# asmirnou/watsor

Measured on AMD Instinct MI355X. Metric: detected frames/sec (whole node) + p50 per-frame latency, SSD-MobileNet 300x300, higher is better.
Workload: dtype f16; 1 GPU; 1 synthetic 640x480 RGB stream per GPU, batch=8 frames, SSD-MobileNet-v2 300x300 (seeded random-init weights), frames resident in HBM, rows copied back to host; batch=8, frame=640x480, parallelism=replica-per-gpu x1, batches_in_flight=4, graph_nodes_per_batch=31

## Files before the change

### include/watsor_hip.h

```cpp
#ifndef WATSOR_HIP_H
#define WATSOR_HIP_H

#include <stdint.h>

#ifdef __cplusplus
extern "C" {
#endif

#define WZ_MAX_DETECTIONS 100
#define WZ_MAX_ZONES 10
#define WZ_NUM_LABELS 91
#define WZ_MAX_CAMS 256

#define WZ_OK 0
#define WZ_EINVAL (-1)
#define WZ_ENOENT (-2)
#define WZ_EFORMAT (-3)
#define WZ_EHIP (-4)
#define WZ_ENODEV (-5)
#define WZ_ELIMIT (-6)
#define WZ_EINCOMPLETE (-7)

typedef struct wz_detection {
    int32_t label;
// ... 102 lines not shown
int wz_input_size(wz_engine_t* e);
int wz_num_anchors(wz_engine_t* e);
int wz_num_classes(wz_engine_t* e);
int wz_precision(wz_engine_t* e);
int wz_hp_blocks(wz_engine_t* e);
double wz_nms_iou(wz_engine_t* e);

int wz_dev_alloc(wz_engine_t* e, uint64_t bytes, void** d_ptr);
int wz_dev_free(wz_engine_t* e, void* d_ptr);
int wz_dev_upload(wz_engine_t* e, void* d_dst, const void* h_src, uint64_t bytes);
int wz_dev_download(wz_engine_t* e, void* h_dst, const void* d_src, uint64_t bytes);

#ifdef WZ_DEV_BUILD
int wz_debug_pyset_order(const int32_t* keys, int n, int32_t* out);
int wz_debug_unused_order(int n, const uint8_t* used, int32_t* out);

int wz_num_tensors(wz_engine_t* e);
int wz_tensor_info(wz_engine_t* e, int idx, char* name, int namelen, int* h, int* w, int* c);
int wz_tensor_flags(wz_engine_t* e, int idx);
int wz_num_ops(wz_engine_t* e);
int wz_op_info(wz_engine_t* e, int idx, char* name, int namelen, int* dims);
int wz_num_stages(wz_engine_t* e);
int wz_stage_name(wz_engine_t* e, int stage, char* name, int namelen);
int wz_profile_device(wz_engine_t* e, int n, const uint8_t* const* d_rgb, const int* w, const int* h,
                      int reps, float* stage_ms);
int wz_profile_stages(wz_engine_t* e, int n, const uint8_t* const* d_rgb, const int* w, const int* h,
                      int reps, int inner, float* stage_ms);

int wz_debug_nms(wz_engine_t* e, int n, uint64_t* out);
int wz_debug_post_lane(wz_engine_t* e, int slot, int n, float* box_enc, float* logits, float* boxes, float* scores,
                       int32_t* classes, int32_t* num, uint64_t* dbg, int32_t* flags);
int wz_debug_mbconv(wz_engine_t* e, uint64_t* out, int32_t* groups);

int wz_debug_lane_stamps(wz_engine_t* e, int slot, uint64_t* out, int cap);
int wz_debug_lane_launch(wz_engine_t* e, int slot, int idx, char* name, int namelen, int* dims);

int wz_stage_preprocess(wz_engine_t* e, const uint8_t* rgb, int w, int h, uint16_t* out_half);
int wz_stage_preprocess_fmt(wz_engine_t* e, const uint8_t* frame, int w, int h, int fmt, uint16_t* out_half);
int wz_stage_forward(wz_engine_t* e, int n, const uint16_t* in_half, float* box_enc, float* logits);
int wz_stage_read_tensor(wz_engine_t* e, int idx, int frame, uint16_t* out_half);
int wz_stage_postprocess(wz_engine_t* e, int n, const float* box_enc, const float* logits, float* boxes,
                         float* scores, int32_t* classes, int32_t* num);
int wz_stage_post_production(wz_engine_t* e, int n, const float* box_enc, const float* logits, int w, int h, wz_detection_t* rows);
int wz_stage_rows(wz_engine_t* e, int w, int h, const float* boxes, const float* scores,
                  const int32_t* classes, wz_detection_t* rows);
int wz_stage_crop_tile(wz_engine_t* e, const uint8_t* frame, int w, int h, int fmt, const wz_tile_t* tile, uint8_t* out);
int wz_stage_merge_tiles(wz_engine_t* e, int w, int h, int cam, int n_tiles, const wz_tile_t* tiles,
                         const wz_detection_t* tile_rows , double iou_thr, double ios_thr,
                         wz_detection_t* rows , uint8_t* pass );
int wz_profile_tiled(wz_engine_t* e, int n, const uint8_t* const* d_frames, const int* w, const int* h, const int* fmt,
                     const int* n_tiles, const wz_tile_t* const* tiles, double iou_thr, double ios_thr, int reps,
                     float* crop_ms, float* merge_ms, float* empty_ms);
int wz_stage_tile_activity(wz_engine_t* e, const uint8_t* frame, int w, int h, int fmt, const wz_tile_t* tile, const uint16_t* ref, int pixel_thr,
                           uint16_t* sums_out, int32_t* changed_out);
int wz_profile_gated(wz_engine_t* e, int n, const uint8_t* const* d_frames, const int* w, const int* h, const int* fmt, const int* cam,
                     double iou_thr, double ios_thr, int reps, float* activity_ms, float* commit_ms, float* empty_ms);
int wz_debug_bound_source(wz_engine_t* e, int slot, int32_t* in_place );

#endif

#ifdef __cplusplus
}
#endif
#endif
```

### watsor_amd/_lib.py

```python
from __future__ import annotations

import ctypes as C
import os

from .share import Detection

_HERE = os.path.dirname(os.path.abspath(__file__))
LIB_PATH = os.path.join(_HERE, "libwatsor_hip.so")
DEV_LIB_PATH = os.environ.get("WATSOR_HIP_DEV_LIBRARY") or os.path.join(_HERE, "libwatsor_hip_dev.so")

WZ_OK, WZ_EINVAL, WZ_ENOENT, WZ_EFORMAT, WZ_EHIP, WZ_ENODEV, WZ_ELIMIT, WZ_EINCOMPLETE = 0, -1, -2, -3, -4, -5, -6, -7
WZ_SLOTS = 8
WZ_FMT_RGB24, WZ_FMT_NV12, WZ_FMT_I420 = 0, 1, 2
WZ_FMT_YUYV422, WZ_FMT_UYVY422, WZ_FMT_GRAY8, WZ_FMT_BGR24 = 3, 4, 5, 6
WZ_FMT_P010, WZ_FMT_YUV420P10 = 0x10, 0x11
WZ_FMT_BASE_MASK, WZ_CSP_BT709, WZ_RANGE_FULL = 0xFF, 0x100, 0x200
WZ_NUM_LABELS = 91
WZ_MAX_CAMS = 256
WZ_MAX_TILES = 64
WZ_GATE_CELL = 16
WZ_SCHEDULE_THROUGHPUT, WZ_SCHEDULE_LATENCY = 0, 1

c_u8p = C.POINTER(C.c_uint8)
c_i32p = C.POINTER(C.c_int32)
# ... 57 lines not shown
    "wz_tracker_count": (C.c_int, [C.c_void_p]),
    "wz_tracker_update": (C.c_int, [C.c_void_p, C.c_void_p, C.c_int, C.c_void_p, C.c_void_p, C.c_int,
                                    C.POINTER(C.c_int), C.POINTER(C.c_int)]),
    "wz_tracker_sieve": (C.c_int, [C.c_void_p, C.c_void_p, C.c_int, C.c_void_p, C.POINTER(C.c_int)]),
    "wz_zones_from_alpha": (C.c_int, [C.c_void_p, C.c_int, C.c_int, C.c_int, C.c_void_p, C.c_void_p]),
    "wz_input_size": (C.c_int, [C.c_void_p]),
    "wz_precision": (C.c_int, [C.c_void_p]),
    "wz_num_anchors": (C.c_int, [C.c_void_p]),
    "wz_num_classes": (C.c_int, [C.c_void_p]),
    "wz_hp_blocks": (C.c_int, [C.c_void_p]),
    "wz_nms_iou": (C.c_double, [C.c_void_p]),
    "wz_dev_alloc": (C.c_int, [C.c_void_p, C.c_uint64, C.POINTER(C.c_void_p)]),
    "wz_dev_free": (C.c_int, [C.c_void_p, C.c_void_p]),
    "wz_dev_upload": (C.c_int, [C.c_void_p, C.c_void_p, C.c_void_p, C.c_uint64]),
    "wz_dev_download": (C.c_int, [C.c_void_p, C.c_void_p, C.c_void_p, C.c_uint64]),
}

DEV_SIGNATURES = {
    "wz_debug_pyset_order": (C.c_int, [C.c_void_p, C.c_int, C.c_void_p]),
    "wz_debug_unused_order": (C.c_int, [C.c_int, C.c_void_p, C.c_void_p]),
    "wz_num_tensors": (C.c_int, [C.c_void_p]),
    "wz_tensor_info": (C.c_int, [C.c_void_p, C.c_int, C.c_char_p, C.c_int, c_i32p, c_i32p, c_i32p]),
    "wz_tensor_flags": (C.c_int, [C.c_void_p, C.c_int]),
    "wz_num_ops": (C.c_int, [C.c_void_p]),
    "wz_op_info": (C.c_int, [C.c_void_p, C.c_int, C.c_char_p, C.c_int, c_i32p]),
    "wz_num_stages": (C.c_int, [C.c_void_p]),
    "wz_stage_name": (C.c_int, [C.c_void_p, C.c_int, C.c_char_p, C.c_int]),
    "wz_profile_device": (C.c_int, [C.c_void_p, C.c_int, C.POINTER(C.c_void_p), c_i32p, c_i32p, C.c_int, c_f32p]),
    "wz_profile_stages": (C.c_int, [C.c_void_p, C.c_int, C.POINTER(C.c_void_p), c_i32p, c_i32p, C.c_int, C.c_int, c_f32p]),
    "wz_debug_nms": (C.c_int, [C.c_void_p, C.c_int, C.c_void_p]),
    "wz_debug_post_lane": (C.c_int, [C.c_void_p, C.c_int, C.c_int, C.c_void_p, C.c_void_p, C.c_void_p, C.c_void_p, C.c_void_p, C.c_void_p,
                                     C.c_void_p, C.c_void_p]),
    "wz_debug_mbconv": (C.c_int, [C.c_void_p, C.c_void_p, C.c_void_p]),
    "wz_debug_lane_stamps": (C.c_int, [C.c_void_p, C.c_int, C.c_void_p, C.c_int]),
    "wz_debug_lane_launch": (C.c_int, [C.c_void_p, C.c_int, C.c_int, C.c_char_p, C.c_int, c_i32p]),
    "wz_stage_preprocess": (C.c_int, [C.c_void_p, C.c_void_p, C.c_int, C.c_int, C.c_void_p]),
    "wz_stage_preprocess_fmt": (C.c_int, [C.c_void_p, C.c_void_p, C.c_int, C.c_int, C.c_int, C.c_void_p]),
    "wz_stage_forward": (C.c_int, [C.c_void_p, C.c_int, C.c_void_p, C.c_void_p, C.c_void_p]),
    "wz_stage_read_tensor": (C.c_int, [C.c_void_p, C.c_int, C.c_int, C.c_void_p]),
    "wz_stage_postprocess": (C.c_int, [C.c_void_p, C.c_int, C.c_void_p, C.c_void_p, C.c_void_p, C.c_void_p,
                                       C.c_void_p, C.c_void_p]),
    "wz_stage_post_production": (C.c_int, [C.c_void_p, C.c_int, C.c_void_p, C.c_void_p, C.c_int, C.c_int, C.c_void_p]),
    "wz_stage_rows": (C.c_int, [C.c_void_p, C.c_int, C.c_int, C.c_void_p, C.c_void_p, C.c_void_p, C.c_void_p]),
    "wz_stage_crop_tile": (C.c_int, [C.c_void_p, C.c_void_p, C.c_int, C.c_int, C.c_int, C.c_void_p, C.c_void_p]),
    "wz_profile_tiled": (C.c_int, [C.c_void_p, C.c_int, C.POINTER(C.c_void_p), c_i32p, c_i32p, c_i32p, c_i32p, C.POINTER(C.c_void_p),
                                   C.c_double, C.c_double, C.c_int, c_f32p, c_f32p, c_f32p]),
    "wz_stage_tile_activity": (C.c_int, [C.c_void_p, C.c_void_p, C.c_int, C.c_int, C.c_int, C.c_void_p, C.c_void_p, C.c_int, C.c_void_p,
                                         C.c_void_p]),
    "wz_profile_gated": (C.c_int, [C.c_void_p, C.c_int, C.POINTER(C.c_void_p), c_i32p, c_i32p, c_i32p, c_i32p, C.c_double, C.c_double, C.c_int,
                                   c_f32p, c_f32p, c_f32p]),
    "wz_debug_bound_source": (C.c_int, [C.c_void_p, C.c_int, C.c_void_p]),
    "wz_stage_merge_tiles": (C.c_int, [C.c_void_p, C.c_int, C.c_int, C.c_int, C.c_int, C.c_void_p, C.c_void_p, C.c_double, C.c_double,
                                       C.c_void_p, C.c_void_p]),
}

_lib = None
_dev_lib = None


class HipLibraryMissing(ImportError):
    pass


class RowsIncomplete(ValueError):
    """WZ_EINCOMPLETE: the call wrote every row, but a frame's rows may be short (clip-after-NMS engines).  The ONLY failure after
    which the rows are valid: callers that must tell "rows written" from "rows not written" catch this class, not ValueError."""
# ... 51 lines not shown
```

### watsor_amd/csrc/k_conv.hip

```cpp
#include "wz_common.h"

__global__ __launch_bounds__(256) void wz_k_stem(const half_t* __restrict__ in, const float* __restrict__ w,
                                                 const float* __restrict__ bias, half_t* __restrict__ out,
                                                 int total, int hin, int win, int hout, int wout, int pad_t,
                                                 int pad_l) {
    __shared__ float sw[27 * 32 + 32];
    for (int i = threadIdx.x; i < 27 * 32; i += 256) sw[i] = w[i];
    if (threadIdx.x < 32) sw[27 * 32 + threadIdx.x] = bias[threadIdx.x];
    __syncthreads();
    const int tid = blockIdx.x * 256 + threadIdx.x;
    if (tid >= total) return;
    const int cg = tid & 3, pix = tid >> 2;
    const int ox = pix % wout;
    const int t2 = pix / wout;
    const int oy = t2 % hout, b = t2 / hout;
    float acc[8];
#pragma unroll
    for (int j = 0; j < 8; ++j) acc[j] = sw[27 * 32 + cg * 8 + j];
#pragma unroll
    for (int ky = 0; ky < 3; ++ky) {
        const int iy = oy * 2 - pad_t + ky;
        if (iy < 0 || iy >= hin) continue;
#pragma unroll
        for (int kx = 0; kx < 3; ++kx) {
// ... 265 lines not shown
    for (int q = q0; q < q1;) {
        wz_conv_load<KS, MT, NT, U>(a, fb, ql, q1, t, c, iy0, ix0, boff, mv, wlane, nt0, cg8);
        wz_conv_mfma(fa, acc);
        q += U;
        if (q >= q1) break;
        wz_conv_load<KS, MT, NT, U>(a, fa, ql, q1, t, c, iy0, ix0, boff, mv, wlane, nt0, cg8);
        wz_conv_mfma(fb, acc);
        q += U;
    }

#pragma unroll
    for (int mt = 0; mt < MT; ++mt) {
        const int m = m_base + mt * 16 + r16;
#pragma unroll
        for (int nt = 0; nt < NT; ++nt) {
            const int n4 = (nt0 + nt) * 16 + g * 4;
            if (a.splitk > 1) {
                if (m < a.M)
                    *reinterpret_cast<float4_t*>(reinterpret_cast<float*>(a.out) +
                                                 ((size_t)bz * a.M + m) * a.n_pad + n4) = acc[mt][nt];
            } else {
                wz_epilogue4(a, m, n4, acc[mt][nt]);
            }
        }
    }
}

template <int KS, int MT, int NT, int U>
__global__ __launch_bounds__(256) void wz_k_conv(const WzConvArgs a) {
    WZ_LANE_STAMP(a.dbg);
    wz_conv_body<KS, MT, NT, U>(a, blockIdx.x, blockIdx.y, blockIdx.z);
}

template <int KS, int WM = 1, int WN = 1, int U = 2, int WGS_PER_CU = 2>
__global__ __launch_bounds__(512, WGS_PER_CU) void wz_k_conv_ws(const WzConvArgs a) {
    WZ_LANE_STAMP(a.dbg);
    constexpr int MT = 2, NT = 2, WAVES = 8, KSPL = WAVES / (WM * WN);
    static_assert(KSPL * WM * WN == WAVES, "eight waves: sub-tiles x K slices");
    __shared__ float4_t red[WAVES][MT * NT][64];
    const int lane = threadIdx.x & 63;
    const int wave = __builtin_amdgcn_readfirstlane(threadIdx.x >> 6);
    const int r16 = lane & 15, g = lane >> 4;
    const int sub = wave / KSPL, ks = wave - sub * KSPL;
    const int m_base = ((int)blockIdx.x * WM + sub / WN) * (MT * 16);
    const int nt0 = ((int)blockIdx.y * WN + sub % WN) * NT;
    const bool tile_live = m_base < a.M && nt0 * 16 < a.n_pad;

    const int hw = a.hout * a.wout;
    int iy0[MT], ix0[MT], boff[MT];
    bool mv[MT];
#pragma unroll
    for (int mt = 0; mt < MT; ++mt) {
        const int m = m_base + mt * 16 + r16;
        mv[mt] = m < a.M;
        const int mm = mv[mt] ? m : 0;
        const int b = mm / hw, rem = mm - b * hw;
        const int oy = rem / a.wout, ox = rem - oy * a.wout;
        iy0[mt] = oy * a.stride - a.pad_t;
        ix0[mt] = ox * a.stride - a.pad_l;
        boff[mt] = b * a.hin;
    }
    float4_t acc[MT][NT];
#pragma unroll
    for (int mt = 0; mt < MT; ++mt)
#pragma unroll
        for (int nt = 0; nt < NT; ++nt) acc[mt][nt] = (float4_t){0.f, 0.f, 0.f, 0.f};

    const int per = (a.kchunks + KSPL - 1) / KSPL;
    const int q0 = ks * per, q1 = min(q0 + per, a.kchunks);
    if (tile_live && q0 < q1) {
        const half_t* wlane = a.w + (size_t)lane * 8;
        const int cg8 = g * 8;
        int ql = q0, t = (KS == 1) ? 0 : q0 / a.kc, c = (KS == 1) ? q0 : q0 - t * a.kc;
        ConvFrags<MT, NT, U> fa, fb;
        wz_conv_load<KS, MT, NT, U>(a, fa, ql, q1, t, c, iy0, ix0, boff, mv, wlane, nt0, cg8);
        for (int q = q0; q < q1;) {
            wz_conv_load<KS, MT, NT, U>(a, fb, ql, q1, t, c, iy0, ix0, boff, mv, wlane, nt0, cg8);
            wz_conv_mfma(fa, acc);
            q += U;
            if (q >= q1) break;
            wz_conv_load<KS, MT, NT, U>(a, fa, ql, q1, t, c, iy0, ix0, boff, mv, wlane, nt0, cg8);
            wz_conv_mfma(fb, acc);
            q += U;
        }
    }
#pragma unroll
    for (int mt = 0; mt < MT; ++mt)
#pragma unroll
        for (int nt = 0; nt < NT; ++nt) red[wave][mt * NT + nt][lane] = acc[mt][nt];
    __syncthreads();
    if (tile_live) {
        for (int tl = ks; tl < MT * NT; tl += KSPL) {
            float4_t v = red[sub * KSPL][tl][lane];
#pragma unroll
            for (int z = 1; z < KSPL; ++z) {
                const float4_t p = red[sub * KSPL + z][tl][lane];
#pragma unroll
                for (int r = 0; r < 4; ++r) v[r] += p[r];
            }
            wz_epilogue4(a, m_base + (tl / NT) * 16 + r16, (nt0 + tl % NT) * 16 + g * 4, v);
        }
    }
}

__global__ __launch_bounds__(256) void wz_k_conv_group(const WzConvGroup g) {
    WZ_LANE_STAMP(g.stamp);
    int e = 0;
    while (e + 1 < g.n && (int)blockIdx.x >= g.first[e + 1]) ++e;
    const int L = (int)blockIdx.x - g.first[e];
    const int gx = g.gx[e], gy = g.gy[e];
    wz_conv_body<3, 2, 2, 4>(g.a[e], L % gx, (L / gx) % gy, L / (gx * gy));
}

__global__ __launch_bounds__(256) void wz_k_splitk_reduce(const WzConvArgs a, const float* __restrict__ ws) {
    WZ_LANE_STAMP(a.dbg);
    const int tid = blockIdx.x * 256 + threadIdx.x;
    const int n4s = a.n_pad >> 2;
// ... 138 lines not shown
void wz_launch_conv(const WzConvArgs& a0, hipStream_t s) {
    if (wz_conv_use_lds(a0)) {
        WzConvArgs a = a0;
        a.grid_m = (a.M + WZ_LDS_TM - 1) / WZ_LDS_TM;
        const int nw = wz_lds_nw(a.M, a.n_pad, a.kchunks);
        a.grid_n = (a.n_pad + WZ_LDS_TN(nw) - 1) / WZ_LDS_TN(nw);
        dim3 grid(a.grid_m * a.grid_n * a.splitk);
        if (nw == 4) {
            if (a.ksize == 1)
                wz_launch_conv_lds<1, 4>(a, grid, s);
            else
                wz_launch_conv_lds<3, 4>(a, grid, s);
        } else {
            if (a.ksize == 1)
                wz_launch_conv_lds<1, 2>(a, grid, s);
            else
                wz_launch_conv_lds<3, 2>(a, grid, s);
        }
        return;
    }
    const WzConvArgs& a = a0;
    if (wz_conv_big(a.M, a.n_pad, a.kchunks))
        wz_launch_conv_cfg<4, 4, 2>(a, s);
    else
        wz_launch_conv_cfg<2, 2, 4>(a, s);
}

bool wz_conv_ws_applies(const WzConvArgs& a) {
    static const int on = wz_dev_env_int("WZ_CONV_WS", 1);
    return on && a.out_mode == WZ_OUT_ACT && a.M <= 1024 && a.kchunks >= 8 && a.n_pad % 32 == 0;
}
void wz_launch_conv_ws(const WzConvArgs& a, hipStream_t s) {
    static const int wide_tiles = wz_dev_env_int("WZ_CONV_WS64", 1);
    if (wide_tiles && a.ksize == 1 && a.M >= 512 && a.n_pad >= 512 && a.n_pad % 64 == 0 && a.kchunks >= 8) {
        WZ_LAUNCH((wz_k_conv_ws<1, 1, 2>), dim3((a.M + 31) / 32, a.n_pad / 64), dim3(512), 0, s, a);
        return;
    }
    const dim3 grid((a.M + 31) / 32, a.n_pad / 32);
    if (a.ksize == 1)
        WZ_LAUNCH(wz_k_conv_ws<1>, grid, dim3(512), 0, s, a);
    else
        WZ_LAUNCH(wz_k_conv_ws<3>, grid, dim3(512), 0, s, a);
}

bool wz_conv_groupable(const WzConvArgs& a) {
    return a.ksize == 3 && !wz_conv_use_lds(a) && !wz_conv_big(a.M, a.n_pad, a.kchunks);
}
void wz_conv_group_add(WzConvGroup& g, const WzConvArgs& a) {
    const int i = g.n++;
    const int mtiles = (a.M + 31) / 32;
    g.a[i] = a;
    g.gx[i] = (mtiles + 3) / 4;
    g.gy[i] = a.n_pad / 32;
    g.first[i + 1] = g.first[i] + g.gx[i] * g.gy[i] * a.splitk;
    g.a[i].grid_m = g.gx[i];
    g.a[i].grid_n = g.gy[i];
}
void wz_launch_conv_group(const WzConvGroup& g, hipStream_t s) {
    WZ_LAUNCH(wz_k_conv_group, dim3(g.first[g.n]), dim3(256), 0, s, g);
}

bool wz_conv_rs_groupable(const WzConvArgs& a) {
    return a.ksize == 3 && wz_conv_use_lds(a);
}
int wz_conv_rs_group_add(WzConvGroup& g, const WzConvArgs& a0) {
    static const int split_n = wz_dev_env_int("WZ_HEAD_SPLIT_N", 1);
    const int nw = wz_lds_nw(a0.M, a0.n_pad, a0.kchunks);
    const bool two = split_n && nw == 4 && (a0.n_pad % 128) == 64 && a0.n_pad > 128;
    if (g.n + (two ? 2 : 1) > WZ_CONV_GROUP_MAX) return 0;
    for (int part = 0; part < (two ? 2 : 1); ++part) {
        const int i = g.n++;
// ... 32 lines not shown
```

### watsor_amd/csrc/k_mbconv_hp.hip

```cpp
#include "wz_common.h"

#include "k_hp_ops.h"

#ifndef WZ_HP_STAMPS
#define WZ_HP_STAMPS 0
#endif
#ifndef WZ_HP_RR3
#define WZ_HP_RR3 1
#endif
#ifndef WZ_HP_ROWS3
#define WZ_HP_ROWS3 1
#endif
#ifndef WZ_HP_STAMP_LAST
#define WZ_HP_STAMP_LAST 0
#endif

template <int NW, bool CS, bool STEM, int MPW, int MQW, int KCI, int NTO, int OCC = 2, bool ONEPASS = false, bool QE = false,
          bool LEAN = false>
__global__ __launch_bounds__(NW * 64, OCC) void wz_k_mbconv_hp(const WzMbArgs a) {
    static_assert(!LEAN || (CS && !ONEPASS && !STEM), "lean: chunk-split");
    static_assert(!LEAN || MQW == 1, "lean builds: 4 x 4 tiles (the 4 x 8 lean builds of round 5 lost their A/B: profiles/r05_blocks_13_16_tile_4x8.txt)");
    extern __shared__ __attribute__((aligned(16))) unsigned char wz_hp_smem[];
    WZ_LANE_STAMP(a.dbg);
    const long long t_entry = WZ_HP_STAMPS ? __builtin_readcyclecounter() : 0;
// ... 18 lines not shown
    const int bidx = (int)blockIdx.x;
    const int nt0 = LEAN ? (bidx % ngrp) * NTO : 0;
    const int wt = LEAN ? bidx / ngrp : CS ? (int)blockIdx.x : (int)blockIdx.x * 4 + __builtin_amdgcn_readfirstlane(wave);
    const bool live = wt < tiles * a.nb;
    const int wtc = live ? wt : 0;
    const int b = wtc / tiles, t = wtc - b * tiles;
    const int tyi = t / a.tiles_x;
    const int oy0 = tyi * a.th, ox0 = (t - tyi * a.tiles_x) * a.tw;
    const int s = a.stride;
    const int hw_ = (a.tw - 1) * s + 3, hh_ = (a.th - 1) * s + 3;
    const int P = hh_ * hw_;
    const int iy_base = oy0 * s - a.pad_t, ix_base = ox0 * s - a.pad_l;
    const half8_t zero8 = {0, 0, 0, 0, 0, 0, 0, 0};

    int hp0[MQW], opix[MQW];
#pragma unroll
    for (int j = 0; j < MQW; ++j) {
        int qy, qx;
        if constexpr (MQW == 2) {
            qx = r16 & 7;
            qy = ((r16 >> 3) << 1) + j;
        } else {
            qy = r16 >> 2;
            qx = r16 & 3;
        }
        hp0[j] = qy * s * hw_ + qx * s;
        const int oy = oy0 + qy, ox = ox0 + qx;
        opix[j] = (live && oy < a.hout && ox < a.wout) ? (b * a.hout + oy) * a.wout + ox : -1;
    }

    half8_t xh[MPW][KCI], xl[MPW][KCI];
    bool inimg[MPW];
    const float rcp_hw = 1.0f / (float)hw_;
#pragma unroll
    for (int i = 0; i < MPW; ++i) {
        const int p = i * 16 + r16;
        const int hy = (int)(((float)p + 0.5f) * rcp_hw), hx = p - hy * hw_;
        const int iy = iy_base + hy, ix = ix_base + hx;
        const bool ok = live && p < P && iy >= 0 && iy < a.hin && ix >= 0 && ix < a.win;
        inimg[i] = ok;
        if constexpr (STEM) {
            auto tap = [&](int tq, bool want) -> half8_t {
                const int ky = tq / 3, kx = tq - ky * 3;
                const int sy = iy * 2 - a.spad_t + ky, sx = ix * 2 - a.spad_l + kx;
                const bool in = want && ok && sy >= 0 && sy < a.sin_h && sx >= 0 && sx < a.sin_w;
                const int cy = min(max(sy, 0), a.sin_h - 1), cx = min(max(sx, 0), a.sin_w - 1);
                const half8_t v = *reinterpret_cast<const half8_t*>(a.in + ((size_t)(b * a.sin_h + cy) * a.sin_w + cx) * 8);
                return in ? v : zero8;
            };
            const half8_t va = tap(2 * g, true), vb = tap(2 * g + 1, true), v8 = tap(8, g <= 1);
            const half_t z16 = (half_t)0.0f;
            const half_t e0h = g == 0 ? v8[0] : g == 1 ? v8[2] : z16, e1h = g == 0 ? v8[1] : z16;
            const half_t e0l = g == 0 ? v8[4] : g == 1 ? v8[6] : z16, e1l = g == 0 ? v8[5] : z16;
            xh[i][0] = (half8_t){va[0], va[1], va[2], e0h, vb[0], vb[1], vb[2], e1h};
            xl[i][0] = (half8_t){va[4], va[5], va[6], e0l, vb[4], vb[5], vb[6], e1l};
        } else if constexpr (!CS) {
            const half_t* src = a.in + ((size_t)(b * a.hin + (ok ? iy : 0)) * a.win + (ok ? ix : 0)) * (2 * a.cin0);
#pragma unroll
            for (int c = 0; c < KCI; ++c) {
                const int k0 = c * 32 + g * 8;
                const bool kok = ok && k0 < a.cin0;
                xh[i][c] = kok ? *reinterpret_cast<const half8_t*>(src + k0) : zero8;
                xl[i][c] = kok ? *reinterpret_cast<const half8_t*>(src + a.cin0 + k0) : zero8;
            }
        }
    }
    constexpr int NFRAG = MPW * KCI * 2;
    unsigned char* const halo_l = wz_hp_smem + REGION + (size_t)a.cmid_pad * (LDSW ? 44 : 8);
    constexpr int PERW = CS ? (NFRAG + NW - 1) / NW : 1;
    half8_t part[PERW];
    if constexpr (CS) {
        static_assert(!STEM, "the stem block runs one wave per tile");
#pragma unroll
        for (int k = 0; k < PERW; ++k) {
            const int f = wave + k * NW;
            part[k] = zero8;
            if (f < NFRAG) {
                const int i = f / (KCI * 2), c = (f >> 1) % KCI, lo = f & 1;
                const int p = i * 16 + r16;
                const int hy = (int)(((float)p + 0.5f) * rcp_hw), hx = p - hy * hw_;
                const int iy = iy_base + hy, ix = ix_base + hx;
                const int k0 = c * 32 + g * 8;
                const bool kok = live && p < P && iy >= 0 && iy < a.hin && ix >= 0 && ix < a.win && k0 < a.cin0;
                const half_t* src = a.in + ((size_t)(b * a.hin + (kok ? iy : 0)) * a.win + (kok ? ix : 0)) * (2 * a.cin0);
                if (kok) part[k] = *reinterpret_cast<const half8_t*>(src + (lo ? a.cin0 : 0) + k0);
            }
        }
    }
    auto park_halo = [&]() {
        if constexpr (CS) {
#pragma unroll
            for (int k = 0; k < PERW; ++k) {
                const int f = wave + k * NW;
                if (f < NFRAG) *reinterpret_cast<half8_t*>(halo_l + (size_t)f * 1024 + lane * 16) = part[k];
            }
        }
    };

    bool interior = true;
#pragma unroll
    for (int i = 0; i < MPW; ++i) interior = interior && __builtin_amdgcn_ballot_w64(!inimg[i] && i * 16 + r16 < P) == 0;

    float4_t acc[MQW][NTO];
#pragma unroll
    for (int j = 0; j < MQW; ++j)
#pragma unroll
        for (int nt = 0; nt < NTO; ++nt) acc[j][nt] = (float4_t){0.f, 0.f, 0.f, 0.f};

    const int nk32 = a.cmid_pad >> 5;
    const int ntiles_e = a.nmid_pad >> 4;
    constexpr int STEP = CS ? NW : 1;
    const int c_lo = 0, c_hi = nk32;
    const int ps0 = CS ? c_lo + wave : 0;
    half8_t wah[2][KCI], wal[2][KCI];
    auto load_wa = [&](int ps) {
#pragma unroll
        for (int nt = 0; nt < 2; ++nt) {
            const int tn = min(ps * 2 + nt, ntiles_e - 1);
            const size_t off = ((size_t)tn * a.kc0 * 64 + lane) * 8;
#pragma unroll
            for (int c = 0; c < KCI; ++c) {
                wah[nt][c] = *reinterpret_cast<const half8_t*>(a.we + off + (size_t)c * 512);
                wal[nt][c] = *reinterpret_cast<const half8_t*>(a.we_lo + off + (size_t)c * 512);
            }
        }
    };
    constexpr bool WA_AHEAD = !((LEAN || !CS) && OCC >= 4);
    if (!CS && WA_AHEAD && ps0 < c_hi) load_wa(ps0);
    {
        constexpr int NT = NW * 64;
        constexpr int WD_IT = LEAN ? (NW >= 8 ? 5 : 9) : 8;
        const int nb4 = a.cmid_pad >> 2;
        float4_t sw[WD_IT], sb, se;
        if constexpr (LDSW) {
// ... 443 lines not shown
    if (a.wout > 19) return -1;
    if (a.stride == 2) return (a.kc0 == 1 && nto == 4) ? HP(6, true, false, 6, 1, 1, 4, 4, false, true, true) : -1;
    if (a.kc0 == 2 && nto == 4) return HP(8, true, false, 3, 1, 2, 4, 4, false, true, true);
    if (a.kc0 == 2 && nto == 6) return HP(8, true, false, 3, 1, 2, 6, 4, false, true, true);
    if (a.kc0 == 3 && nto == 6) return HP(8, true, false, 3, 1, 3, 6, 4, false, true, true);
    return -1;
}

constexpr int HP_CS_FEW_WGS = 64;
constexpr int HP_CS_S1_MAX_W = 38;
static int wz_hp_pick(const WzMbArgs& a, int n, hipStream_t s, bool prepare, bool few) {
    const int nto = a.n_pad / 16, nk32 = a.cmid_pad >> 5;
    if (a.stem) return (a.kc0 == 1 && nto == 2 && a.stride == 1) ? HP(4, false, true, 4, 2, 1, 2, 3) : -1;
    if (a.cin0 == 0) return -1;
    if (a.wout > 19 && a.kc0 == 1 && nto == 2) {
        const bool cs = ((a.stride == 1 && a.wout <= HP_CS_S1_MAX_W) || few) && nk32 >= 4 && nk32 <= 6;
        if (a.stride == 2) return (cs && nk32 <= 5) ? HP(5, true, false, 6, 1, 1, 2, 2) : HP(4, false, false, 6, 1, 1, 2, 3);
        if (cs && a.wout <= 38) return nk32 <= 5 ? HP(5, true, false, 4, 2, 1, 2, 4) : HP(6, true, false, 4, 2, 1, 2, 4);
        if (cs) return HP(3, true, false, 4, 2, 1, 2, 2);
        return a.wout >= 75 ? HP(4, false, false, 4, 2, 1, 2, 3) : HP(4, false, false, 4, 2, 1, 2, 2);
    }
    if (a.wout > 19) return -1;
    if (a.stride == 2) return (a.kc0 == 1 && nto == 4) ? HP(6, true, false, 6, 1, 1, 4, 4, false, false, true) : -1;
    if (a.kc0 == 2 && nto == 4) return HP(8, true, false, 3, 1, 2, 4, 4, false, false, true);
    if (a.kc0 == 2 && nto == 6) return HP(8, true, false, 3, 1, 2, 6, 4, false, false, true);
    if (a.kc0 == 3 && nto == 6) return HP(8, true, false, 3, 1, 3, 6, 4, false, false, true);
    return -1;
}
#undef HP

int wz_launch_mbconv_hp(const WzMbArgs& a0, int n, hipStream_t s, bool prepare) {
    WzMbArgs a = a0;
    a.nsplit = 1;
    if (a.nmid_pad != a.cmid_pad || (a.cmid_pad & 31) || a.kc != (a.cmid_pad >> 5) || !a.we_lo || !a.wp_lo) return -1;
    if (a.qenc) {
        if (!prepare) return wz_hp_pick_q(a, n, s, false, wz_hp_small_batch("WZ_HP_SMALL_CS", n), wz_hp_small_batch("WZ_HP_TILES44", n));
        int r = 0;
        for (int v = 0; v < 4; ++v) r |= wz_hp_pick_q(a, n, s, true, v & 1, v >> 1);
        return r;
    }
    if (!a.stem && a.cin0 != 0 && a.wout <= 10) return prepare ? wz_launch_mbconv_hp2(a, n, s, true, 0) : -1;
    const int tiles_s1 = ((a.hout + 3) / 4) * ((a.wout + (a.stride == 1 ? 7 : 3)) / (a.stride == 1 ? 8 : 4));
    auto few = [&](int nb) { return (tiles_s1 * nb + 3) / 4 <= HP_CS_FEW_WGS; };
    if (!prepare) return wz_hp_pick(a, n, s, false, few(n));
    return wz_hp_pick(a, n, s, true, few(1)) | wz_hp_pick(a, n, s, true, few(4095));
}
```

### watsor_amd/csrc/wz_common.h

```cpp
#pragma once
#include <hip/hip_runtime.h>
#include <hip/hip_fp16.h>
#include <stdint.h>
#include <stdlib.h>

#include "../../include/watsor_hip.h"
#include "wz_program.h"

typedef _Float16 half_t;
typedef __attribute__((ext_vector_type(8))) _Float16 half8_t;
typedef __attribute__((ext_vector_type(4))) _Float16 half4_t;
typedef __attribute__((ext_vector_type(4))) float float4_t;
#ifdef __HIPCC__
__device__ __forceinline__ half4_t wz_relu6_pack(const float4_t d, const float4_t bv, bool keep) {
    typedef __attribute__((ext_vector_type(2))) unsigned int wz_uint2_t;
    half4_t o;
#pragma unroll
    for (int r = 0; r < 4; ++r) o[r] = (half_t)fminf(fmaxf(d[r] + bv[r], 0.0f), 6.0f);
    wz_uint2_t p = __builtin_bit_cast(wz_uint2_t, o);
    p[0] = keep ? p[0] : 0u;
    p[1] = keep ? p[1] : 0u;
    return __builtin_bit_cast(half4_t, p);
}
#endif
// ... 44 lines not shown
    int32_t clip_after;
    int32_t _pad;
};

struct WzMbArgs {
    const half_t* in;
    const half_t* we;
    const float* be;
    const half_t* wd;
    const float* bd;
    const half_t* wp;
    const float* bp;
    const half_t* res;
    half_t* out;
    int32_t hin, win, hout, wout;
    int32_t cin0, kc0, nmid_pad;
    int32_t cmid, cmid_pad, kc;
    int32_t cout, n_pad;
    int32_t stride, pad_t, pad_l;
    int32_t stem, sin_h, sin_w, spad_t, spad_l;
    float* ws;
    uint64_t ws_bytes;
    int32_t M;
    unsigned long long* dbg;
    int32_t th, tw, tiles_y, tiles_x, nsplit, cpg, stage, ebufs, nb;
    const half_t* we_lo;
    const half_t* wp_lo;
    int32_t hp, hp_out;
    half_t* out2;
    int32_t has_out2;
    int32_t qenc;
    unsigned long long* dbg2;
    int32_t lone;
};

struct WzDwsepArgs {
    const half_t* in;
    const half_t* wd;
    const float* bd;
    const half_t* wp;
    const float* bp;
    half_t* out;
    int32_t M;
    int32_t hin, win, hout, wout;
    int32_t cin, kc, cout, n_pad;
    int32_t stride, pad_t, pad_l;
    unsigned long long* dbg;
};

struct WzCamFilter {
    int32_t enabled, width, height, n_zones;
    const int32_t* sat;
    double conf_thr[WZ_NUM_LABELS];
    double area_thr[WZ_NUM_LABELS];
    uint8_t allow[WZ_NUM_LABELS][WZ_MAX_ZONES * 4];
};
#define WZ_MAX_ZONES_PER_CAM (WZ_MAX_ZONES * 4)


extern thread_local int wz_launch_repeat;
static inline const char* wz_dev_getenv(const char* name) {
#ifdef WZ_DEV_BUILD
    return getenv(name);
#else
    (void)name;
    return nullptr;
#endif
}
static inline int wz_dev_env_int(const char* name, int dflt) {
    const char* e = wz_dev_getenv(name);
    return (e && e[0] && atoi(e) >= 0) ? atoi(e) : dflt;
}

bool wz_latency_schedule();

#ifndef WZ_LANE_STAMPS
#define WZ_LANE_STAMPS 0
#endif
#define WZ_STAMP_SLOTS 128
#define WZ_STAMP_WORDS 384
#define WZ_STAMP_ENTRY 16
#define WZ_STAMP_EXIT 80
#define WZ_STAMP_PRE_BYTES (WZ_STAMP_WORDS * 8)
struct WzLaunchNote { const void* func; unsigned grid[3], block[3]; unsigned lds; };
#if WZ_LANE_STAMPS
void wz_note_launch(const void* func, dim3 grid, dim3 block, size_t lds);
#define WZ_LAUNCH(kern, grid, block, lds, s, ...) do { wz_note_launch(reinterpret_cast<const void*>(kern), grid, block, lds); \
        for (int _wz_r = 0; _wz_r < wz_launch_repeat; ++_wz_r) hipLaunchKernelGGL(kern, grid, block, lds, s, __VA_ARGS__); } while (0)
#ifdef __HIPCC__
struct WzLaneStamp {
    unsigned long long* p;
    __device__ __forceinline__ explicit WzLaneStamp(unsigned long long* q) : p(q) {
        if (p && threadIdx.x == 0 && threadIdx.y == 0 && threadIdx.z == 0) {
            const unsigned id = blockIdx.x + gridDim.x * (blockIdx.y + gridDim.y * blockIdx.z);
            if (id < 64u) p[WZ_STAMP_ENTRY + id] = (unsigned long long)wall_clock64();
        }
    }
    __device__ __forceinline__ ~WzLaneStamp() {
        if (p && threadIdx.x == 0 && threadIdx.y == 0 && threadIdx.z == 0) {
            const unsigned id = blockIdx.x + gridDim.x * (blockIdx.y + gridDim.y * blockIdx.z);
            p[WZ_STAMP_EXIT + (id & 255u)] = (unsigned long long)wall_clock64();
        }
    }
};
// ... 163 lines not shown
```

### watsor_amd/csrc/wz_engine.hip

```cpp
#include <math.h>
#include <stdarg.h>
#include <stdio.h>
#include <stdlib.h>
#include <string.h>

#include <algorithm>
#include <atomic>
#include <chrono>

#include "wz_engine.h"

static const char kHwQueuesVar[] = "GPU_MAX_HW_QUEUES";
static const int kHwQueuesNeeded = 8;
static int wz_env_hw_queues() {
    const char* v = getenv(kHwQueuesVar);
    if (!v || !v[0]) return 0;
    char* end = nullptr;
    const long n = strtol(v, &end, 10);
    while (*end == ' ' || *end == '\t') ++end;
    return (*end || n < 1 || n > 1 << 20) ? 0 : (int)n;
}
#ifndef WZ_KEEP_HOST_HW_QUEUES
__attribute__((constructor)) static void wz_runtime_defaults() {
    if (wz_env_hw_queues() < kHwQueuesNeeded) setenv(kHwQueuesVar, "8", 1);
// ... 1471 lines not shown

extern "C" int wz_debug_post_lane(wz_engine_t* e, int slot, int n, float* box_enc, float* logits, float* boxes, float* scores,
                                  int32_t* classes, int32_t* num, uint64_t* dbg, int32_t* flags) {
    if (!e || slot < 0 || slot >= e->n_lanes || n < 1 || n > e->max_batch) return wz_fail(WZ_EINVAL, "wz_debug_post_lane: bad argument");
    HIPCHK(hipSetDevice(e->device));
    const Lane& L = e->lanes[slot];
    HIPCHK(hipStreamSynchronize(L.stream));
    const size_t A = e->hdr.num_anchors, C = e->hdr.num_classes, T = e->hdr.max_total;
    if (T != WZ_MAX_DETECTIONS) return wz_fail(WZ_EINVAL, "wz_debug_post_lane: max_total %zu, expected %d", T, WZ_MAX_DETECTIONS);
    if (box_enc) HIPCHK(hipMemcpy(box_enc, L.d_box_enc, n * A * 16, hipMemcpyDeviceToHost));
    if (logits) HIPCHK(hipMemcpy(logits, L.d_logits, n * A * C * 4, hipMemcpyDeviceToHost));
    if (boxes) HIPCHK(hipMemcpy(boxes, L.post.det_boxes, n * T * 16, hipMemcpyDeviceToHost));
    if (scores) HIPCHK(hipMemcpy(scores, L.post.det_scores, n * T * 4, hipMemcpyDeviceToHost));
    if (classes) HIPCHK(hipMemcpy(classes, L.post.det_classes, n * T * 4, hipMemcpyDeviceToHost));
    if (num) HIPCHK(hipMemcpy(num, L.post.det_num, (size_t)n * 4, hipMemcpyDeviceToHost));
    if (dbg) HIPCHK(hipMemcpy(dbg, L.post.dbg, (size_t)n * 16 * 8, hipMemcpyDeviceToHost));
    if (flags) {
        const auto it = L.post_modes.find(L.key);
        flags[0] = it == L.post_modes.end() ? 0 : it->second & 1;
        flags[1] = it == L.post_modes.end() ? 0 : (it->second >> 1) & 1;
    }
    return WZ_OK;
}

extern "C" int wz_debug_mbconv(wz_engine_t* e, uint64_t* out, int32_t* groups) {
    if (!e || !out || !e->d_mbdbg) return wz_fail(WZ_EINVAL, "wz_debug_mbconv: create the engine with WZ_MB_DEBUG=1");
    HIPCHK(hipSetDevice(e->device));
    WZCHK(sync_all(e));
    HIPCHK(hipMemcpy(out, e->d_mbdbg, (size_t)e->hdr.n_ops * 16 * 8, hipMemcpyDeviceToHost));
    if (groups) memcpy(groups, e->mb_groups.data(), sizeof(int) * e->hdr.n_ops);
    return WZ_OK;
}

extern "C" int wz_debug_lane_stamps(wz_engine_t* e, int slot, uint64_t* out, int cap) {
#if WZ_LANE_STAMPS
    if (!e || !out || slot < 0 || slot >= e->n_lanes) return wz_fail(WZ_EINVAL, "wz_debug_lane_stamps: bad argument");
    const Lane& L = e->lanes[slot];
    const int k = L.post.stamps_n;
    if (!L.h_stamps || k <= 0 || cap < k + 1) return wz_fail(WZ_EINVAL, "wz_debug_lane_stamps: no stamped batch on lane %d (or cap %d < %d)", slot, cap, k + 1);
    for (int i = 0; i < 2 * k; ++i) out[i] = L.h_stamps[i];
    uint64_t t0 = ~0ull, t1 = 0;
    for (int f = 0; f < L.n; ++f) {
        t0 = std::min<uint64_t>(t0, L.h_stamps[2 * (k + f)]);
        t1 = std::max<uint64_t>(t1, L.h_stamps[2 * (k + f) + 1]);
    }
    out[2 * k] = t0;
    out[2 * k + 1] = t1;
    return k + 1;
#else
    (void)e; (void)slot; (void)out; (void)cap;
    return wz_fail(WZ_EINVAL, "wz_debug_lane_stamps: this library was not built with -DWZ_LANE_STAMPS=1 (`make stamps`)");
#endif
}
extern "C" int wz_debug_lane_launch(wz_engine_t* e, int slot, int idx, char* name, int namelen, int* dims) {
#if WZ_LANE_STAMPS
    if (!e || slot < 0 || slot >= e->n_lanes || !dims) return wz_fail(WZ_EINVAL, "wz_debug_lane_launch: bad argument");
    Lane& L = e->lanes[slot];
    auto it = L.launch_notes.find(L.key);
    if (it == L.launch_notes.end() || idx < 0 || idx >= (int)it->second.size()) return wz_fail(WZ_EINVAL, "wz_debug_lane_launch: no launch %d", idx);
    const WzLaunchNote& ln = it->second[idx];
    HIPCHK(hipSetDevice(e->device));
    const char* nm = hipKernelNameRefByPtr(ln.func, L.stream);
    if (name && namelen > 0) snprintf(name, namelen, "%s", nm ? nm : "?");
    hipFuncAttributes fa;
    memset(&fa, 0, sizeof(fa));
    (void)hipFuncGetAttributes(&fa, ln.func);
// ... 260 lines not shown
```

Measured before the change: 49480 frames/s.

## Add specialized pointwise-conv loader and direct stem gather fast paths

Adds a pointwise (1x1, stride 1, no pad) specialization of the workspace conv kernel. It loads activations as contiguous rows with pointer increments instead of computing im2col coordinates per chunk, and doubles the occupancy hint in launch bounds. It also adds a stem fast path in the fused mbconv kernel that gathers 3x3 stride-2 input taps with direct vector loads when the tile is fully interior, skipping the general bounds-checked gather and the interior ballot. Both paths can be disabled through a dev-only mask for comparison. The cost is extra code paths and higher register pressure limits that could cause spills.

```diff
diff --git a/include/watsor_hip.h b/include/watsor_hip.h
--- a/include/watsor_hip.h
+++ b/include/watsor_hip.h
@@ -158,6 +158,8 @@
                        int32_t* classes, int32_t* num, uint64_t* dbg, int32_t* flags);
 int wz_debug_mbconv(wz_engine_t* e, uint64_t* out, int32_t* groups);
 
+int wz_debug_general_paths(int mask);
+
 int wz_debug_lane_stamps(wz_engine_t* e, int slot, uint64_t* out, int cap);
 int wz_debug_lane_launch(wz_engine_t* e, int slot, int idx, char* name, int namelen, int* dims);
 
diff --git a/watsor_amd/_lib.py b/watsor_amd/_lib.py
--- a/watsor_amd/_lib.py
+++ b/watsor_amd/_lib.py
@@ -113,6 +113,7 @@
     "wz_debug_post_lane": (C.c_int, [C.c_void_p, C.c_int, C.c_int, C.c_void_p, C.c_void_p, C.c_void_p, C.c_void_p, C.c_void_p, C.c_void_p,
                                      C.c_void_p, C.c_void_p]),
     "wz_debug_mbconv": (C.c_int, [C.c_void_p, C.c_void_p, C.c_void_p]),
+    "wz_debug_general_paths": (C.c_int, [C.c_int]),
     "wz_debug_lane_stamps": (C.c_int, [C.c_void_p, C.c_int, C.c_void_p, C.c_int]),
     "wz_debug_lane_launch": (C.c_int, [C.c_void_p, C.c_int, C.c_int, C.c_char_p, C.c_int, c_i32p]),
     "wz_stage_preprocess": (C.c_int, [C.c_void_p, C.c_void_p, C.c_int, C.c_int, C.c_void_p]),
diff --git a/watsor_amd/csrc/k_conv.hip b/watsor_amd/csrc/k_conv.hip
--- a/watsor_amd/csrc/k_conv.hip
+++ b/watsor_amd/csrc/k_conv.hip
@@ -321,11 +321,12 @@
     wz_conv_body<KS, MT, NT, U>(a, blockIdx.x, blockIdx.y, blockIdx.z);
 }
 
-template <int KS, int WM = 1, int WN = 1, int U = 2, int WGS_PER_CU = 2>
-__global__ __launch_bounds__(512, WGS_PER_CU) void wz_k_conv_ws(const WzConvArgs a) {
+template <int KS, int WM = 1, int WN = 1, int U = 2, int WGS_PER_CU = 2, bool PW = false>
+__global__ __launch_bounds__(512, PW ? 2 * WGS_PER_CU : WGS_PER_CU) void wz_k_conv_ws(const WzConvArgs a) {
     WZ_LANE_STAMP(a.dbg);
     constexpr int MT = 2, NT = 2, WAVES = 8, KSPL = WAVES / (WM * WN);
     static_assert(KSPL * WM * WN == WAVES, "eight waves: sub-tiles x K slices");
+    static_assert(!PW || KS == 1, "pointwise loader: 1x1");
     __shared__ float4_t red[WAVES][MT * NT][64];
     const int lane = threadIdx.x & 63;
     const int wave = __builtin_amdgcn_readfirstlane(threadIdx.x >> 6);
@@ -335,6 +336,85 @@
     const int nt0 = ((int)blockIdx.y * WN + sub % WN) * NT;
     const bool tile_live = m_base < a.M && nt0 * 16 < a.n_pad;
 
+    float4_t acc[MT][NT];
+#pragma unroll
+    for (int mt = 0; mt < MT; ++mt)
+#pragma unroll
+        for (int nt = 0; nt < NT; ++nt) acc[mt][nt] = (float4_t){0.f, 0.f, 0.f, 0.f};
+
+    const int per = (a.kchunks + KSPL - 1) / KSPL;
+    const int q0 = ks * per, q1 = min(q0 + per, a.kchunks);
+    if constexpr (PW) {
+        if (tile_live && q0 < q1) {
+            const int cg8 = g * 8;
+            const half_t* xp[MT];
+            const half_t* wp[NT];
+#pragma unroll
+            for (int mt = 0; mt < MT; ++mt) {
+                const int m = m_base + mt * 16 + r16;
+                xp[mt] = a.in + (size_t)(m < a.M ? m : 0) * a.cin + q0 * 32 + cg8;
+            }
+#pragma unroll
+            for (int nt = 0; nt < NT; ++nt) wp[nt] = a.w + ((size_t)(nt0 + nt) * a.kc + q0) * 512 + (size_t)lane * 8;
+            const half8_t zero = {0, 0, 0, 0, 0, 0, 0, 0};
+            const int whole = min(q1, a.cin >> 5) - q0;
+            const int nfull = whole > 0 ? whole / U : 0;
+            const int ql_tail = q0 + nfull * U;
+            auto load_full = [&](ConvFrags<MT, NT, U>& f) {
+#pragma unroll
+                for (int u = 0; u < U; ++u) {
+#pragma unroll
+                    for (int mt = 0; mt < MT; ++mt) f.xa[u][mt] = *reinterpret_cast<const half8_t*>(xp[mt] + u * 32);
+#pragma unroll
+                    for (int nt = 0; nt < NT; ++nt) f.wf[u][nt] = *reinterpret_cast<const half8_t*>(wp[nt] + u * 512);
+                }
+#pragma unroll
+                for (int mt = 0; mt < MT; ++mt) xp[mt] += U * 32;
+#pragma unroll
+                for (int nt = 0; nt < NT; ++nt) wp[nt] += U * 512;
+            };
+            int ql = ql_tail;
+            auto load_edge = [&](ConvFrags<MT, NT, U>& f) {
+#pragma unroll
+                for (int u = 0; u < U; ++u) {
+                    const bool live = ql + u < q1;
+                    const bool x_ok = live && ((ql + u + 1) * 32 <= a.cin || (ql + u) * 32 + cg8 < a.cin);
+#pragma unroll
+                    for (int mt = 0; mt < MT; ++mt) f.xa[u][mt] = x_ok ? *reinterpret_cast<const half8_t*>(xp[mt] + u * 32) : zero;
+#pragma unroll
+                    for (int nt = 0; nt < NT; ++nt) f.wf[u][nt] = live ? *reinterpret_cast<const half8_t*>(wp[nt] + u * 512) : zero;
+                }
+                ql += U;
+#pragma unroll
+                for (int mt = 0; mt < MT; ++mt) xp[mt] += U * 32;
+#pragma unroll
+                for (int nt = 0; nt < NT; ++nt) wp[nt] += U * 512;
+            };
+            ConvFrags<MT, NT, U> fa, fb;
+            if (nfull > 0) {
+                load_full(fa);
+                const int pairs = (nfull - 1) >> 1;
+                for (int p = 0; p < pairs; ++p) {
+                    load_full(fb);
+                    wz_conv_mfma(fa, acc);
+                    load_full(fa);
+                    wz_conv_mfma(fb, acc);
+                }
+                ql -= ((nfull - 1) & 1) * U;
+                const int more = (q1 - ql + U - 1) / U;
+                if (more >= 1) load_edge(fb);
+                wz_conv_mfma(fa, acc);
+                if (more >= 1) {
+                    if (more >= 2) load_edge(fa);
+                    wz_conv_mfma(fb, acc);
+                    if (more >= 2) wz_conv_mfma(fa, acc);
+                }
+            } else {
+                load_edge(fa);
+                wz_conv_mfma(fa, acc);
+            }
+        }
+    } else {
     const int hw = a.hout * a.wout;
     int iy0[MT], ix0[MT], boff[MT];
     bool mv[MT];
@@ -349,14 +429,6 @@
         ix0[mt] = ox * a.stride - a.pad_l;
         boff[mt] = b * a.hin;
     }
-    float4_t acc[MT][NT];
-#pragma unroll
-    for (int mt = 0; mt < MT; ++mt)
-#pragma unroll
-        for (int nt = 0; nt < NT; ++nt) acc[mt][nt] = (float4_t){0.f, 0.f, 0.f, 0.f};
-
-    const int per = (a.kchunks + KSPL - 1) / KSPL;
-    const int q0 = ks * per, q1 = min(q0 + per, a.kchunks);
     if (tile_live && q0 < q1) {
         const half_t* wlane = a.w + (size_t)lane * 8;
         const int cg8 = g * 8;
@@ -372,6 +444,7 @@
             wz_conv_mfma(fb, acc);
             q += U;
         }
+    }
     }
 #pragma unroll
     for (int mt = 0; mt < MT; ++mt)
@@ -576,11 +649,20 @@
 }
 void wz_launch_conv_ws(const WzConvArgs& a, hipStream_t s) {
     static const int wide_tiles = wz_dev_env_int("WZ_CONV_WS64", 1);
+    const bool pw = !wz_general_path(WZ_GENERAL_CONV_LOADER) && a.ksize == 1 && a.stride == 1 && a.pad_t == 0 && a.pad_l == 0 && a.hin == a.hout && a.win == a.wout;
     if (wide_tiles && a.ksize == 1 && a.M >= 512 && a.n_pad >= 512 && a.n_pad % 64 == 0 && a.kchunks >= 8) {
-        WZ_LAUNCH((wz_k_conv_ws<1, 1, 2>), dim3((a.M + 31) / 32, a.n_pad / 64), dim3(512), 0, s, a);
+        const dim3 grid((a.M + 31) / 32, a.n_pad / 64);
+        if (pw)
+            WZ_LAUNCH((wz_k_conv_ws<1, 1, 2, 2, 2, true>), grid, dim3(512), 0, s, a);
+        else
+            WZ_LAUNCH((wz_k_conv_ws<1, 1, 2>), grid, dim3(512), 0, s, a);
         return;
     }
     const dim3 grid((a.M + 31) / 32, a.n_pad / 32);
+    if (pw) {
+        WZ_LAUNCH((wz_k_conv_ws<1, 1, 1, 2, 2, true>), grid, dim3(512), 0, s, a);
+        return;
+    }
     if (a.ksize == 1)
         WZ_LAUNCH(wz_k_conv_ws<1>, grid, dim3(512), 0, s, a);
     else
diff --git a/watsor_amd/csrc/k_mbconv_hp.hip b/watsor_amd/csrc/k_mbconv_hp.hip
--- a/watsor_amd/csrc/k_mbconv_hp.hip
+++ b/watsor_amd/csrc/k_mbconv_hp.hip
@@ -74,6 +74,34 @@
     half8_t xh[MPW][KCI], xl[MPW][KCI];
     bool inimg[MPW];
     const float rcp_hw = 1.0f / (float)hw_;
+    bool stem_fast = false;
+    if constexpr (STEM) {
+        const int sy0 = iy_base * 2 - a.spad_t, sx0 = ix_base * 2 - a.spad_l;
+        stem_fast = live && !a.stem_general && iy_base >= 0 && iy_base + hh_ <= a.hin && ix_base >= 0 && ix_base + hw_ <= a.win &&
+                    sy0 >= 0 && sy0 + (hh_ - 1) * 2 + 2 < a.sin_h && sx0 >= 0 && sx0 + (hw_ - 1) * 2 + 2 < a.sin_w;
+        if (stem_fast) {
+            const unsigned char* const base = reinterpret_cast<const unsigned char*>(a.in + ((size_t)(b * a.sin_h + sy0) * a.sin_w + sx0) * 8);
+            const int ta = 2 * g, tb = 2 * g + 1;
+            const unsigned offa = (unsigned)((ta / 3) * a.sin_w + ta % 3) * 16u, offb = (unsigned)((tb / 3) * a.sin_w + tb % 3) * 16u;
+            const unsigned off8 = (unsigned)(2 * a.sin_w + 2) * 16u;
+            const half_t z16 = (half_t)0.0f;
+#pragma unroll
+            for (int i = 0; i < MPW; ++i) {
+                const int p = min(i * 16 + r16, P - 1);
+                const int hy = (int)(((float)p + 0.5f) * rcp_hw), hx = p - hy * hw_;
+                const unsigned o = (unsigned)(hy * 2 * a.sin_w + hx * 2) * 16u;
+                const half8_t va = *reinterpret_cast<const half8_t*>(base + (o + offa));
+                const half8_t vb = *reinterpret_cast<const half8_t*>(base + (o + offb));
+                const half8_t v8 = *reinterpret_cast<const half8_t*>(base + (o + off8));
+                const half_t e0h = g == 0 ? v8[0] : g == 1 ? v8[2] : z16, e1h = g == 0 ? v8[1] : z16;
+                const half_t e0l = g == 0 ? v8[4] : g == 1 ? v8[6] : z16, e1l = g == 0 ? v8[5] : z16;
+                xh[i][0] = (half8_t){va[0], va[1], va[2], e0h, vb[0], vb[1], vb[2], e1h};
+                xl[i][0] = (half8_t){va[4], va[5], va[6], e0l, vb[4], vb[5], vb[6], e1l};
+                inimg[i] = true;
+            }
+        }
+    }
+    if (!stem_fast) {
 #pragma unroll
     for (int i = 0; i < MPW; ++i) {
         const int p = i * 16 + r16;
@@ -107,6 +135,7 @@
             }
         }
     }
+    }
     constexpr int NFRAG = MPW * KCI * 2;
     unsigned char* const halo_l = wz_hp_smem + REGION + (size_t)a.cmid_pad * (LDSW ? 44 : 8);
     constexpr int PERW = CS ? (NFRAG + NW - 1) / NW : 1;
@@ -140,8 +169,10 @@
     };
 
     bool interior = true;
-#pragma unroll
-    for (int i = 0; i < MPW; ++i) interior = interior && __builtin_amdgcn_ballot_w64(!inimg[i] && i * 16 + r16 < P) == 0;
+    if (!stem_fast) {
+#pragma unroll
+        for (int i = 0; i < MPW; ++i) interior = interior && __builtin_amdgcn_ballot_w64(!inimg[i] && i * 16 + r16 < P) == 0;
+    }
 
     float4_t acc[MQW][NTO];
 #pragma unroll
@@ -651,6 +682,7 @@
 int wz_launch_mbconv_hp(const WzMbArgs& a0, int n, hipStream_t s, bool prepare) {
     WzMbArgs a = a0;
     a.nsplit = 1;
+    a.stem_general = wz_general_path(WZ_GENERAL_STEM_GATHER);
     if (a.nmid_pad != a.cmid_pad || (a.cmid_pad & 31) || a.kc != (a.cmid_pad >> 5) || !a.we_lo || !a.wp_lo) return -1;
     if (a.qenc) {
         if (!prepare) return wz_hp_pick_q(a, n, s, false, wz_hp_small_batch("WZ_HP_SMALL_CS", n), wz_hp_small_batch("WZ_HP_TILES44", n));
diff --git a/watsor_amd/csrc/wz_common.h b/watsor_amd/csrc/wz_common.h
--- a/watsor_amd/csrc/wz_common.h
+++ b/watsor_amd/csrc/wz_common.h
@@ -100,6 +100,7 @@
     int32_t qenc;
     unsigned long long* dbg2;
     int32_t lone;
+    int32_t stem_general;
 };
 
 struct WzDwsepArgs {
@@ -138,6 +139,18 @@
 static inline int wz_dev_env_int(const char* name, int dflt) {
     const char* e = wz_dev_getenv(name);
     return (e && e[0] && atoi(e) >= 0) ? atoi(e) : dflt;
+}
+
+#define WZ_GENERAL_STEM_GATHER 1
+#define WZ_GENERAL_CONV_LOADER 2
+static inline bool wz_general_path(int bit) {
+#ifdef WZ_DEV_BUILD
+    extern int wz_general_paths_mask;
+    return (wz_general_paths_mask & bit) != 0;
+#else
+    (void)bit;
+    return false;
+#endif
 }
 
 bool wz_latency_schedule();
diff --git a/watsor_amd/csrc/wz_engine.hip b/watsor_amd/csrc/wz_engine.hip
--- a/watsor_amd/csrc/wz_engine.hip
+++ b/watsor_amd/csrc/wz_engine.hip
@@ -1527,6 +1527,13 @@
     return WZ_OK;
 }
 
+int wz_general_paths_mask = 0;
+extern "C" int wz_debug_general_paths(int mask) {
+    const int before = wz_general_paths_mask;
+    if (mask >= 0) wz_general_paths_mask = mask & 3;
+    return before;
+}
+
 extern "C" int wz_debug_lane_stamps(wz_engine_t* e, int slot, uint64_t* out, int cap) {
 #if WZ_LANE_STAMPS
     if (!e || !out || slot < 0 || slot >= e->n_lanes) return wz_fail(WZ_EINVAL, "wz_debug_lane_stamps: bad argument");
```

Result: no change. 49870 frames/s, median of 6 (+0.8%).
